# s-a-malik/fumi

Measured on AMD Instinct MI355X. Metric: episodes/sec (5-way 5-shot FuMI), higher is better.
Workload: dtype f32; 1 GPU; FuMI 5-way 5-shot, 32 query/class, ResNet-152-style 2048-d embeddings, im_hid [256,64], GloVe-300 token text (L=128, V=20000, mean pool), text_hid 256, 1 inner step, second-order meta-gradient + Adam step; BASELINE.json configs[1]; episodes_per_gpu=32, global_meta_batch=32, parallelism=episode-sharded x1, 1 all-reduce of the flat gradient

## Files before the change

fumi_amd/csrc/episode.hip:

```cpp
#include "common.h"
#include <algorithm>
#include <stdlib.h>

namespace {

unsigned long long* g_epi_trace = nullptr;
int g_spin_limit = 1 << 22;
constexpr int QR = 32;
constexpr int MAXL = FUMI_MAX_HIDDEN;

struct EpiBuf {
    float *A0, *G;
    float *D, *cs;
    float *bcur[MAXL], *bh;
    float *Wslot[MAXL], *Whslot;
    float *ta[MAXL], *tdz[MAXL], *tp, *te;
    float *lg;
    float *aq[MAXL], *zq[MAXL], *lbar, *qcs;
    float *pW[MAXL], *pb[MAXL], *pWh, *pbh, *pb0, *pD, *ploss, *pcorr;
    float *Wb[MAXL], *bb[MAXL], *Whb, *bhb, *b0b, *Db;
    float *abar[MAXL], *X0, *X1, *eb, *lb;
    float *A0bar;
    float *A0bar_q; int ldsr, ldq;
    float *apart; int *acnt;
// ... 950 lines not shown
    float* Whb = w.Whb + (long)b * N * H;
    float* bhb = w.bhb + (long)b * N;
    float* b0b = w.b0b + (long)b * h0;
    float* Db = w.Db + (long)b * S * h0;
    float* A0bs = w.A0bar + (long)b * w.ldsr * h0;
    auto sum_tiles = [&](float* dst, const float* src, long sz) {
        wg_sum_slabs(dst, src + (long)b * ntile * sz, ntile, sz, sz);
    };
    for (int i = 1; i < L; ++i) {
        const long sz = (long)d.h[i] * d.h[i - 1];
        sum_tiles(Wb(i), w.pW[i], sz);
        sum_tiles(bb(i), w.pb[i], d.h[i]);
    }
    sum_tiles(Whb, w.pWh, (long)N * H);
    sum_tiles(bhb, w.pbh, N);
    sum_tiles(b0b, w.pb0, h0);
    sum_tiles(Db, w.pD, (long)S * h0);
    for (int i = tid; i < S * h0; i += nt) A0bs[i] = 0.f;
    __syncthreads();

    if (d.second_order) {
        const float* Gss = w.G + (long)b * (S + d.Qn) * S;
        float* cs = w.cs + (long)b * h0;
        float* eb = w.eb + (long)b * S * N;
        float* lb = w.lb + (long)b * S * N;
        float* const Xa = w.X0 + (long)b * S * w.maxh;
        float* const Xb = w.X1 + (long)b * S * w.maxh;
        auto X = [&](int i) { return i ? Xb : Xa; };
        for (int t = d.T - 1; t >= 0; --t) {
            auto a = [&](int i) { return (const float*)(w.ta[i] + ((long)b * w.ntape + t) * S * d.h[i]); };
            auto dz = [&](int i) { return (const float*)(w.tdz[i] + ((long)b * w.ntape + t) * S * d.h[i]); };
            auto ab = [&](int i) { return w.abar[i] + (long)b * S * d.h[i]; };
            auto Wc = [&](int i) { return (const float*)(w.Wslot[i] + ((long)b * w.nslot + t) * ((long)d.h[i] * d.h[i - 1])); };
            const float* Whc = w.Whslot + ((long)b * w.nslot + t) * N * H;
            const float* p = w.tp + ((long)b * w.ntape + t) * S * N;
            const float* e = w.te + ((long)b * w.ntape + t) * S * N;

            for (int i = 0; i < L; ++i) {
                float* abi = ab(i);
                for (int j = tid; j < S * d.h[i]; j += nt) abi[j] = 0.f;
            }
            int cur = 0;
            {
                wg_ew((long)S * h0, Xa, a(0), Db, nullptr, [&](long, float m_, float v, float) { return m_ > 0.f ? v * d.mscale : 0.f; });
            }
            __syncthreads();
            for (int i = 1; i < L; ++i) {
                const int hi = d.h[i], hp = d.h[i - 1];
                const float* dab = X(cur); float* nxt = X(cur ^ 1);
                const float* bbi = bb(i); const float* Wbi = Wb(i); const float* ai = a(i);
                wg_mm2(sm, sm_cap, S, hi, hp, dab, hp, 1, Wc(i), 1, hp, [&](int m, int n) { return bbi[n]; },
                       [&](int m, int n, float acc, float pre) { nxt[(long)m * hi + n] = acc - alpha * pre; });
                wg_mm2(sm, sm_cap, S, hi, hp, a(i - 1), hp, 1, Wbi, 1, hp,
                       [&](int m, int n) { return f32pair{nxt[(long)m * hi + n], ai[(long)m * hi + n]}; },
                       [&](int m, int n, float acc, f32pair pre) {
                           nxt[(long)m * hi + n] = pre.y > 0.f ? (pre.x - alpha * acc) * d.mscale : 0.f;
                       });
                float* abp = ab(i - 1);
                wg_mm2(sm, sm_cap, S, hp, hi, dz(i), hi, 1, Wbi, hp, 1, [&](int m, int n) { return abp[(long)m * hp + n]; },
                       [&](int m, int n, float acc, float pre) { abp[(long)m * hp + n] = pre - alpha * acc; });
                __syncthreads();
                float* Wbw = Wb(i);
                wg_mm2(sm, sm_cap, hi, hp, S, dz(i), 1, hi, dab, hp, 1, [&](int m, int n) { return Wbw[(long)m * hp + n]; },
                       [&](int m, int n, float acc, float pre) { Wbw[(long)m * hp + n] = pre + acc; });
                __syncthreads();
                cur ^= 1;
            }
            {
                const float* dab = X(cur);
                wg_mm2(sm, sm_cap, S, N, H, dab, H, 1, Whc, 1, H, [&](int m, int n) { return bhb[n]; },
                       [&](int m, int n, float acc, float pre) { eb[m * N + n] = acc - alpha * pre; });
                wg_mm2(sm, sm_cap, S, N, H, a(L - 1), H, 1, Whb, 1, H, [&](int m, int n) { return eb[m * N + n]; },
                       [&](int m, int n, float acc, float pre) { eb[m * N + n] = pre - alpha * acc; });
                float* abl = ab(L - 1);
                wg_mm2(sm, sm_cap, S, H, N, e, N, 1, Whb, H, 1, [&](int m, int n) { return abl[(long)m * H + n]; },
                       [&](int m, int n, float acc, float pre) { abl[(long)m * H + n] = pre - alpha * acc; });
                __syncthreads();
                wg_mm2(sm, sm_cap, N, H, S, e, 1, N, dab, H, 1, [&](int m, int n) { return Whb[m * H + n]; },
                       [&](int m, int n, float acc, float pre) { Whb[m * H + n] = pre + acc; });
                for (int s = tid; s < S; s += nt) {
                    float dot = 0.f;
                    for (int n = 0; n < N; ++n) dot += p[s * N + n] * eb[s * N + n];
                    for (int n = 0; n < N; ++n) lb[s * N + n] = p[s * N + n] * (eb[s * N + n] - dot) / (float)S;
                }
                __syncthreads();
                wg_mm2(sm, sm_cap, S, H, N, lb, N, 1, Whc, H, 1, [&](int m, int n) { return abl[(long)m * H + n]; },
                       [&](int m, int n, float acc, float pre) { abl[(long)m * H + n] = pre + acc; });
                wg_mm2(sm, sm_cap, N, H, S, lb, 1, N, a(L - 1), H, 1, [&](int m, int n) { return Whb[m * H + n]; },
                       [&](int m, int n, float acc, float pre) { Whb[m * H + n] = pre + acc; });
                wg_colsum(sm, sm_cap, S, N, lb, N, [&](int n, float s) { bhb[n] += s; });
                __syncthreads();
            }
            for (int i = L - 1; i >= 1; --i) {
                const int hi = d.h[i], hp = d.h[i - 1];
                float* zb = ab(i);
                {
                    wg_ew((long)S * hi, zb, a(i), zb, nullptr, [&](long, float m_, float v, float) { return m_ > 0.f ? v * d.mscale : 0.f; });
                }
                __syncthreads();
                float* abp = ab(i - 1); float* Wbw = Wb(i); float* bbw = bb(i);
                wg_mm2(sm, sm_cap, S, hp, hi, zb, hi, 1, Wc(i), hp, 1, [&](int m, int n) { return abp[(long)m * hp + n]; },
                       [&](int m, int n, float acc, float pre) { abp[(long)m * hp + n] = pre + acc; });
                wg_mm2(sm, sm_cap, hi, hp, S, zb, 1, hi, a(i - 1), hp, 1, [&](int m, int n) { return Wbw[(long)m * hp + n]; },
                       [&](int m, int n, float acc, float pre) { Wbw[(long)m * hp + n] = pre + acc; });
                wg_colsum(sm, sm_cap, S, hi, zb, hi, [&](int n, float s) { bbw[n] += s; });
                __syncthreads();
            }
            float* z0b = ab(0);
            wg_ew((long)S * h0, z0b, a(0), z0b, nullptr, [&](long, float m_, float v, float) { return m_ > 0.f ? v * d.mscale : 0.f; });
            __syncthreads();
            wg_ew((long)S * h0, A0bs, A0bs, z0b, nullptr, [&](long, float x, float y, float) { return x + y; });
            __syncthreads();
            wg_colsum(sm, sm_cap, S, h0, z0b, h0, [&](int n, float s) { cs[n] = s; b0b[n] += s; });
            __syncthreads();
            wg_mm2(sm, sm_cap, S, h0, S, Gss, S, 1, z0b, h0, 1,
                   [&](int m, int n) { return f32pair{Db[(long)m * h0 + n], cs[n]}; },
                   [&](int m, int n, float acc, f32pair pre) { Db[(long)m * h0 + n] = pre.x - alpha * (acc + pre.y); });
            __syncthreads();
        }
    }
    float* hb = head_bar + (long)b * N * (H + 1);
    for (int j = tid; j < N * H; j += nt) hb[(j / H) * (H + 1) + (j % H)] = Whb[j];
    for (int j = tid; j < N; j += nt) hb[j * (H + 1) + H] = bhb[j];
}

constexpr int RLDS_CAP = 40000;
struct RLay {
    int Wb[MAXL], bb[MAXL], a[MAXL], dz[MAXL], W[MAXL], ab[MAXL];
    int Db, A0bs, b0b, Whb, bhb, Wh, p, e, eb, G, dab0, X0, X1, cs, ldX, total;
};
__host__ __device__ constexpr void reverse_layout(RLay& y, int L, const int* h, int S, int N, int P) {
    int off = 0;
    const int RS = q_r4(S), h0c = h[0] / P, H = h[L - 1];
    auto take = [&](int rows, int ld) { const int o = off; off += rows * ld; return o; };
    for (int i = 0; i < MAXL; ++i) y.Wb[i] = y.bb[i] = y.a[i] = y.dz[i] = y.W[i] = y.ab[i] = 0;
    int maxh1 = 4;
    for (int i = 1; i < L; ++i) maxh1 = h[i] > maxh1 ? h[i] : maxh1;
    y.ldX = wg_ld(maxh1);
    for (int i = 1; i < L; ++i) {
        const int kc = i == 1 ? h0c : h[i - 1];
        y.Wb[i] = take(q_r16(h[i]), wg_ld(kc)); y.W[i] = take(q_r16(h[i]), wg_ld(kc)); y.bb[i] = take(1, q_r4(h[i]));
        y.a[i] = take(RS, wg_ld(h[i])); y.dz[i] = take(RS, wg_ld(h[i])); y.ab[i] = take(RS, wg_ld(h[i]));
    }
    y.a[0] = take(RS, wg_ld(h0c)); y.ab[0] = take(RS, wg_ld(h0c)); y.dab0 = take(RS, wg_ld(h0c));
    y.Db = take(RS, wg_ld(h0c)); y.A0bs = take(RS, wg_ld(h0c));
    y.X0 = take(RS, y.ldX); y.X1 = take(RS, y.ldX);
    y.Whb = take(q_r16(N), wg_ld(H)); y.Wh = take(q_r16(N), wg_ld(H));
    y.p = take(RS, wg_ld(N)); y.e = take(RS, wg_ld(N)); y.eb = take(RS, wg_ld(N)); y.G = take(RS, wg_ld(S));
    y.b0b = take(1, q_r4(h0c)); y.cs = take(1, q_r4(h0c)); y.bhb = take(1, q_r4(N));
    y.total = off + 64;
}
constexpr RLay ref_rlay() { RLay y{}; const int h[MAXL] = {REF_H0, REF_H1}; reverse_layout(y, 2, h, REF_SP, REF_NP, REF_P); return y; }
static_assert(ref_qlay().total <= QLDS_CAP && ref_rlay().total <= RLDS_CAP, "the reference layouts fit the CU's LDS");

template <bool FIX = false, bool DROP = true>
__global__ __launch_bounds__(512) void reverse_lds_kernel(StageTab stg_init, StageTab stg_step, EpiDims d_arg, EpiBuf w, RLay y_arg,
                                                          int P_arg, float* loss_b, float* acc_b, float* head_bar) {
    EpiDims d_fix = d_arg; fix_dims<FIX, DROP>(d_fix);
    const EpiDims& d = FIX ? d_fix : d_arg;
    auto dh = [&](int i) { return FIX ? (i == 0 ? REF_H0 : REF_H1) : d_arg.h[i]; };
    RLay y_fix = y_arg;
    if constexpr (FIX) { constexpr RLay k = ref_rlay(); y_fix = k; }
    const RLay& y = FIX ? y_fix : y_arg;
    const int P = FIX ? REF_P : P_arg;
    extern __shared__ __attribute__((aligned(16))) float sm[];
    __shared__ StageTab s_stg[2];
    const int tid = threadIdx.x, nt = blockDim.x;
    const int xcd = blockIdx.x & 7, jq = blockIdx.x >> 3;
    const int b = xcd + 8 * (jq / P), c = jq % P;
    if (b >= d.B) return;
    int ri = 0;
#define RSTAMP() if (w.trace && tid == 0 && blockIdx.x == 0) w.trace[128 + ri++] = __builtin_amdgcn_s_memrealtime();
    RSTAMP()
    const int S = d.S, N = d.N, L = d.L, H = d.H, h0 = dh(0), h0c = h0 / P, c0 = c * h0c, h1 = dh(1);
    const float alpha = d.alpha, ms = d.mscale;
    const int ntile = w.ntile;
    if (tid == 0 && c == 0) {
        float ls = 0.f, cr = 0.f;
        for (int t = 0; t < ntile; ++t) { ls += w.ploss[(long)b * ntile + t]; cr += w.pcorr[(long)b * ntile + t]; }
        loss_b[b] = ls / (float)d.Qn;
        acc_b[b] = cr / (float)d.Qn;
    }
    if (!d.need_grad) return;

    const int ldc = wg_ld(h0c), ldN = wg_ld(N), ldS = wg_ld(S), ldH = wg_ld(H), ldX = y.ldX;
    auto ldh = [&](int i) { return wg_ld(dh(i)); };
    const f32x4 z4 = {0.f, 0.f, 0.f, 0.f};
    auto relu_bwd4 = [&](const f32x4& act, const f32x4& g) {
        f32x4 o;
#pragma unroll
        for (int e = 0; e < 4; ++e) o[e] = act[e] > 0.f ? g[e] * ms : 0.f;
        return o;
    };
    auto ew = [&](int cols, auto&& f) {
        const int c4n = (cols + 3) >> 2;
        for (int i = tid; i < S * c4n; i += nt) { const int m = i / c4n; f(m, (i - m * c4n) << 2); }
    };
    auto store_img = [&](float* dst, long drs, const float* img, int ld, int rows, int cols) {
        const int c4n = (cols + 3) >> 2;
        for (int i = tid; i < rows * c4n; i += nt) {
            const int r = i / c4n, cc = (i - r * c4n) << 2;
            wg_st4(dst + (long)r * drs + cc, *(const f32x4*)(img + r * ld + cc), min(4, cols - cc));
        }
    };

    wg_stage_tab_to_lds(s_stg, 2, (int)(2 * sizeof(StageTab) + sizeof(EpiDims) + sizeof(EpiBuf) + sizeof(RLay) + 64));
    for (int i = tid * 4, tot = y.total; i < tot; i += nt * 4) *(f32x4*)(sm + i) = z4;
    __syncthreads(); RSTAMP()
    wg_stage_rows<3, 8>(&s_stg[0], b, 0, c, 0, sm);
    wg_lds_barrier(); RSTAMP()

    float* Wb1 = sm + y.Wb[1]; float* Db = sm + y.Db; float* A0bs = sm + y.A0bs; float* b0b = sm + y.b0b;
    float* Whb = sm + y.Whb; float* bhb = sm + y.bhb; float* cs = sm + y.cs;
    float* a0 = sm + y.a[0]; float* ab0 = sm + y.ab[0]; float* dab0 = sm + y.dab0; float* W1 = sm + y.W[1];
    float* Wh = sm + y.Wh; float* pp = sm + y.p; float* ee = sm + y.e; float* eb = sm + y.eb; float* G = sm + y.G;
    float* Xa = sm + y.X0; float* Xb = sm + y.X1;

    if (d.second_order) {
        for (int t = d.T - 1; t >= 0; --t) {
            const int round = d.T - 1 - t;
            wg_stage_rows<8, 1>(&s_stg[1], b, t, c, 0, sm);
            wg_lds_barrier(); RSTAMP()
            for (int i = 1; i < L; ++i) { float* abi = sm + y.ab[i]; const int ldi = ldh(i); ew(dh(i), [&](int m, int n) { *(f32x4*)(abi + m * ldi + n) = z4; }); }
            ew(h0c, [&](int m, int n) {
                *(f32x4*)(ab0 + m * ldc + n) = z4;
                *(f32x4*)(dab0 + m * ldc + n) = relu_bwd4(*(const f32x4*)(a0 + m * ldc + n), *(const f32x4*)(Db + m * ldc + n));
            });
            wg_lds_barrier(); RSTAMP()
            const float* dz1 = sm + y.dz[1]; const int ld1 = ldh(1);
            wg_lmm<true, true>(S, h1, h0c, dab0, ldc, W1, ldc, [&](int m, int n, const f32x4& acc, int) { *(f32x4*)(Xa + m * ldX + n) = acc; });
            wg_lmm<true, true>(S, h1, h0c, a0, ldc, Wb1, ldc, [&](int m, int n, const f32x4& acc, int) {
                float* px = Xa + m * ldX + n; *(f32x4*)px = *(const f32x4*)px - alpha * acc;
            });
            wg_lmm_wide<true>(S, h0c, h1, dz1, ld1, Wb1, ldc, [&](int m, int n, const f32x4& acc, int, auto) {
                float* pa = ab0 + m * ldc + n; *(f32x4*)pa = *(const f32x4*)pa - alpha * acc;
            });
            wg_lds_barrier(); RSTAMP()
            float* xb = w.xpart + (((long)b * 2 + (round & 1)) * 8) * (long)S * h1;
            if (P > 1) {
                float* mine = xb + (long)c * S * h1;
                for (int i = tid; i < S * h1; i += nt) {
                    const int m = i / h1, n = i - m * h1;
                    __hip_atomic_store(mine + i, Xa[m * ldX + n], __ATOMIC_RELAXED, __HIP_MEMORY_SCOPE_AGENT);
                }
            }
            wg_lmm_wide<false>(h1, h0c, S, dz1, ld1, dab0, ldc, [&](int m, int n, const f32x4& acc, int, auto) {
                float* pw = Wb1 + m * ldc + n; *(f32x4*)pw = *(const f32x4*)pw + acc;
            });
            if (P > 1) {
                wg_drain_stores();
                __syncthreads();
                if (tid == 0) {
                    __hip_atomic_fetch_add(w.xcnt + b, 1, __ATOMIC_RELAXED, __HIP_MEMORY_SCOPE_AGENT);
                    const int target = P * (round + 1);
                    int spin = 0;
                    while (__hip_atomic_load(w.xcnt + b, __ATOMIC_RELAXED, __HIP_MEMORY_SCOPE_AGENT) < target) {
                        if (++spin > w.spin_limit) { atomicOr(w.status, FUMI_ST_SYNC_TIMEOUT); break; }
                        __builtin_amdgcn_s_sleep(2);
                    }
                }
                __syncthreads();
            } else {
                wg_lds_barrier();
            }
            RSTAMP()
            {
                const float* a1 = sm + y.a[1]; const float* bb1 = sm + y.bb[1];
                const int w4 = q_r4(h1);
                for (int i = tid; i < S * w4; i += nt) {
                    const int m = i / w4, n = i - m * w4;
                    float v = 0.f;
                    if (n < h1) {
                        if (P > 1) { for (int cc = 0; cc < P; ++cc) v += __hip_atomic_load(xb + (long)cc * S * h1 + m * h1 + n, __ATOMIC_RELAXED, __HIP_MEMORY_SCOPE_AGENT); }
                        else v = Xa[m * ldX + n];
                        v = a1[m * ld1 + n] > 0.f ? (v - alpha * bb1[n]) * ms : 0.f;
                    }
                    Xb[m * ldX + n] = v;
                }
            }
            wg_lds_barrier(); RSTAMP()
            int cur = 1;
            auto X = [&](int i) { return i ? Xb : Xa; };
            for (int i = 2; i < L; ++i) {
                const int hi = dh(i), hp = dh(i - 1), ldi = ldh(i), ldp = ldh(i - 1);
                const float* dab = X(cur); float* nxt = X(cur ^ 1);
                const float* bbi = sm + y.bb[i]; float* Wbi = sm + y.Wb[i]; const float* ai = sm + y.a[i];
                const float* dzi = sm + y.dz[i]; float* abp = sm + y.ab[i - 1];
                wg_lmm<true, true>(S, hi, hp, dab, ldX, sm + y.W[i], ldp, [&](int m, int n, const f32x4& acc, int) {
                    *(f32x4*)(nxt + m * ldX + n) = acc - alpha * *(const f32x4*)(bbi + n);
                });
                wg_lmm<true, true>(S, hi, hp, sm + y.a[i - 1], ldp, Wbi, ldp, [&](int m, int n, const f32x4& acc, int) {
                    float* px = nxt + m * ldX + n;
                    *(f32x4*)px = relu_bwd4(*(const f32x4*)(ai + m * ldi + n), *(const f32x4*)px - alpha * acc);
                });
                wg_lmm_wide<true>(S, hp, hi, dzi, ldi, Wbi, ldp, [&](int m, int n, const f32x4& acc, int, auto) {
                    float* pa = abp + m * ldp + n; *(f32x4*)pa = *(const f32x4*)pa - alpha * acc;
                });
                wg_lds_barrier();
                wg_lmm_wide<false>(hi, hp, S, dzi, ldi, dab, ldX, [&](int m, int n, const f32x4& acc, int, auto) {
                    float* pw = Wbi + m * ldp + n; *(f32x4*)pw = *(const f32x4*)pw + acc;
                });
                wg_lds_barrier();
                cur ^= 1;
            }
            {
                const float* dab = X(cur); const float* aL = sm + y.a[L - 1]; float* abl = sm + y.ab[L - 1];
                wg_lmm<true, true>(S, N, H, dab, ldX, Wh, ldH, [&](int m, int n, const f32x4& acc, int) {
                    *(f32x4*)(eb + m * ldN + n) = acc - alpha * *(const f32x4*)(bhb + n);
                });
                wg_lmm<true, true>(S, N, H, aL, ldH, Whb, ldH, [&](int m, int n, const f32x4& acc, int) {
                    float* pe = eb + m * ldN + n; *(f32x4*)pe = *(const f32x4*)pe - alpha * acc;
                });
                wg_lmm_wide<true>(S, H, N, ee, ldN, Whb, ldH, [&](int m, int n, const f32x4& acc, int, auto) {
                    float* pa = abl + m * ldH + n; *(f32x4*)pa = *(const f32x4*)pa - alpha * acc;
                });
                wg_lds_barrier(); RSTAMP()
                wg_lmm_wide<false>(N, H, S, ee, ldN, dab, ldX, [&](int m, int n, const f32x4& acc, int, auto) {
                    float* pw = Whb + m * ldH + n; *(f32x4*)pw = *(const f32x4*)pw + acc;
                });
                for (int s_ = tid; s_ < S; s_ += nt) {
                    float* re = eb + s_ * ldN; const float* rp = pp + s_ * ldN;
                    float dot = 0.f;
                    for (int n = 0; n < N; ++n) dot += rp[n] * re[n];
                    for (int n = 0; n < N; ++n) re[n] = rp[n] * (re[n] - dot) / (float)S;
                    for (int n = N; n < q_r4(N); ++n) re[n] = 0.f;
                }
                wg_lds_barrier(); RSTAMP()
                const float* lb = eb;
                wg_lmm_wide<true>(S, H, N, lb, ldN, Wh, ldH, [&](int m, int n, const f32x4& acc, int, auto) {
                    float* pa = abl + m * ldH + n; *(f32x4*)pa = *(const f32x4*)pa + acc;
                });
                wg_lmm_wide<false>(N, H, S, lb, ldN, aL, ldH, [&](int m, int n, const f32x4& acc, int, auto) {
                    float* pw = Whb + m * ldH + n; *(f32x4*)pw = *(const f32x4*)pw + acc;
                });
                wg_lcolsum(S, N, lb, ldN, [&](int n, float s_) { bhb[n] += s_; });
                wg_lds_barrier(); RSTAMP()
            }
            for (int i = L - 1; i >= 1; --i) {
                const int hi = dh(i), ldi = ldh(i);
                float* zb = sm + y.ab[i]; const float* ai = sm + y.a[i];
                ew(hi, [&](int m, int n) { float* pz = zb + m * ldi + n; *(f32x4*)pz = relu_bwd4(*(const f32x4*)(ai + m * ldi + n), *(const f32x4*)pz); });
                wg_lds_barrier();
                float* bbw = sm + y.bb[i];
                if (i >= 2) {
                    const int hp = dh(i - 1), ldp = ldh(i - 1);
                    float* abp = sm + y.ab[i - 1]; float* Wbi = sm + y.Wb[i];
                    wg_lmm_wide<true>(S, hp, hi, zb, ldi, sm + y.W[i], ldp, [&](int m, int n, const f32x4& acc, int, auto) {
                        float* pa = abp + m * ldp + n; *(f32x4*)pa = *(const f32x4*)pa + acc;
                    });
                    wg_lmm_wide<false>(hi, hp, S, zb, ldi, sm + y.a[i - 1], ldp, [&](int m, int n, const f32x4& acc, int, auto) {
                        float* pw = Wbi + m * ldp + n; *(f32x4*)pw = *(const f32x4*)pw + acc;
                    });
                } else {
                    wg_lmm_wide<true>(S, h0c, hi, zb, ldi, W1, ldc, [&](int m, int n, const f32x4& acc, int, auto) {
                        float* pa = ab0 + m * ldc + n; *(f32x4*)pa = *(const f32x4*)pa + acc;
                    });
                    wg_lmm_wide<false>(hi, h0c, S, zb, ldi, a0, ldc, [&](int m, int n, const f32x4& acc, int, auto) {
                        float* pw = Wb1 + m * ldc + n; *(f32x4*)pw = *(const f32x4*)pw + acc;
                    });
                }
                wg_lcolsum(S, hi, zb, ldi, [&](int n, float s_) { bbw[n] += s_; });
                wg_lds_barrier(); RSTAMP()
            }
            ew(h0c, [&](int m, int n) {
                float* pz = ab0 + m * ldc + n;
                const f32x4 z = relu_bwd4(*(const f32x4*)(a0 + m * ldc + n), *(const f32x4*)pz);
                *(f32x4*)pz = z;
                float* pA = A0bs + m * ldc + n; *(f32x4*)pA = *(const f32x4*)pA + z;
            });
            wg_lds_barrier();
            wg_lcolsum(S, h0c, ab0, ldc, [&](int n, float s_) { cs[n] = s_; b0b[n] += s_; });
            wg_lds_barrier();
            wg_lmm_wide<true>(S, h0c, S, G, ldS, ab0, ldc, [&](int m, int n, const f32x4& acc, int, auto) {
                float* pd = Db + m * ldc + n; *(f32x4*)pd = *(const f32x4*)pd - alpha * (acc + *(const f32x4*)(cs + n));
            });
            wg_lds_barrier(); RSTAMP()
        }
    }
    store_img(w.Wb[1] + (long)b * h1 * h0 + c0, h0, Wb1, ldc, h1, h0c);
    store_img(w.A0bar + (long)b * w.ldsr * h0 + c0, h0, A0bs, ldc, S, h0c);
    for (int n = tid; n < h0c; n += nt) w.b0b[(long)b * h0 + c0 + n] = b0b[n];
    if (c == 0) {
        for (int i = 1; i < L; ++i) {
            const float* bbi = sm + y.bb[i];
            for (int n = tid; n < dh(i); n += nt) w.bb[i][(long)b * dh(i) + n] = bbi[n];
            if (i >= 2) store_img(w.Wb[i] + (long)b * dh(i) * dh(i - 1), dh(i - 1), sm + y.Wb[i], ldh(i - 1), dh(i), dh(i - 1));
        }
        float* hb = head_bar + (long)b * N * (H + 1);
        for (int j = tid; j < N * H; j += nt) { const int n = j / H, k = j - n * H; hb[n * (H + 1) + k] = Whb[n * ldH + k]; }
        for (int j = tid; j < N; j += nt) hb[j * (H + 1) + H] = bhb[j];
    }
    RSTAMP()
#undef RSTAMP
}

__global__ void class_text_select_kernel(int N, int S, int Dt, const float* text_s, const int64_t* y_s, float* out,
                                         int* status) {
    const int b = blockIdx.y, n = blockIdx.x, lane = threadIdx.x;
    const int64_t* ys = y_s + (long)b * S;
    int first = S;
    for (int s0 = 0; s0 < S && first == S; s0 += 64) {
        const int s = s0 + lane;
        const bool hit = s < S && ys[s] == n;
        const unsigned long long m = __ballot(hit);
        if (m) first = s0 + __ffsll((long long)m) - 1;
    }
    float* o = out + ((long)b * N + n) * Dt;
    if (first == S) {
        if (lane == 0) atomicOr(status, FUMI_ST_CLASS_MISSING);
        for (int j = lane; j < Dt; j += 64) o[j] = __builtin_nanf("");
        return;
    }
    const float* src = text_s + ((long)b * S + first) * Dt;
    for (int j = lane; j < Dt; j += 64) o[j] = src[j];
}

__global__ void broadcast_head_kernel(int N, int H, const float* Wf, const float* bf, float* head) {
    float* hb = head + (long)blockIdx.x * N * (H + 1);
    for (int j = threadIdx.x; j < N * (H + 1); j += blockDim.x) {
        const int n = j / (H + 1), c = j % (H + 1);
        hb[j] = c < H ? Wf[n * H + c] : bf[n];
    }
}

__global__ void tanh_bwd_kernel(long n, const float* h, const float* hbar, float* out) {
    for (long i = blockIdx.x * (long)blockDim.x + threadIdx.x; i < n; i += (long)gridDim.x * blockDim.x)
        out[i] = hbar[i] * (1.f - h[i] * h[i]);
}

__global__ void relu_mask_mul_kernel(long n, const float* u, float* g, float scale) {
    for (long i = blockIdx.x * (long)blockDim.x + threadIdx.x; i < n; i += (long)gridDim.x * blockDim.x)
        g[i] = u[i] > 0.f ? g[i] * scale : 0.f;
}

__global__ void split_head_grad_kernel(int B, int N, int H, const float* head_bar, float scale, float* gW, float* gb) {
    const int j = blockIdx.x * blockDim.x + threadIdx.x;
    if (j >= N * (H + 1)) return;
    float s = 0.f;
    for (int b = 0; b < B; ++b) s += head_bar[(long)b * N * (H + 1) + j];
    const int n = j / (H + 1), c = j % (H + 1);
    if (c < H) gW[n * H + c] = scale * s; else gb[n] = scale * s;
}

template <auto K> struct KernTag { static constexpr auto fn = K; };

inline int blocks_for(long n) { long b = (n + 255) / 256; return (int)(b > 2048 ? 2048 : (b < 1 ? 1 : b)); }

struct Carver {
    fumi_ws* ws; size_t bytes;
    float* take(size_t n) {
        bytes += ws_align(n * sizeof(float));
        return ws ? ws_f(ws, n) : nullptr;
    }
};

void carve(Carver& c, const EpisodeProblem& p, EpiBuf& w) {
    const size_t B = p.B, S = p.S, Qn = p.Qn, N = p.N, L = p.L, h0 = p.h[0], H = p.h[L - 1];
    const bool taped = p.need_grad && p.second_order && p.T > 0;
    w.nslot = taped ? p.T + 1 : 1;
    w.ntape = taped ? p.T : 1;
    w.ntile = (p.Qn + QR - 1) / QR;
    int maxh = 0;
    for (int i = 0; i < p.L; ++i) maxh = p.h[i] > maxh ? p.h[i] : maxh;
    w.maxh = maxh;
    {
        auto r16 = [](int x) { return (x + 15) & ~15; };
        auto need = [&](int M, int N_, int K) { return (long)(r16(M) + 4 + r16(N_) + 4) * (r16(K) + 4); };
        const int S_ = p.S, N_ = p.N, H_ = p.h[p.L - 1], h0_ = p.h[0], R_ = QR;
        long a = need(S_, h0_, S_), q = need(R_, h0_, S_), r = need(S_, h0_, S_);
        a = std::max({a, need(S_, N_, H_), need(S_, H_, N_), need(N_, H_, S_)});
        q = std::max({q, need(R_, N_, H_), need(N_, H_, R_), need(R_, H_, N_), need(S_, h0_, R_)});
        r = std::max({r, need(S_, N_, H_), need(S_, H_, N_), need(N_, H_, S_)});
        for (int i = 1; i < p.L; ++i) {
            const int hi = p.h[i], hp = p.h[i - 1];
            a = std::max({a, need(S_, hi, hp), need(S_, hp, hi), need(hi, hp, S_)});
            q = std::max({q, need(R_, hi, hp), need(R_, hp, hi), need(hi, hp, R_)});
            r = std::max({r, need(S_, hi, hp), need(S_, hp, hi), need(hi, hp, S_)});
        }
        const long cap = 38000;
        w.lds_adapt = (int)std::min(a, cap); w.lds_query = (int)std::min(q, cap); w.lds_reverse = (int)std::min(r, cap);
    }
    const size_t nt = w.ntile;
    w.A0 = c.take(B * (S + Qn) * h0); w.G = c.take(B * (S + Qn) * S);
    w.D = c.take(B * S * h0); w.cs = c.take(B * h0);
    w.bh = c.take(B * N); w.Whslot = c.take(B * w.nslot * N * H);
    w.tp = c.take(B * w.ntape * S * N); w.te = c.take(B * w.ntape * S * N);
    w.lg = c.take(B * S * N);
    w.lbar = c.take(B * Qn * N); w.qcs = c.take(B * nt * h0);
    w.ploss = c.take(B * nt); w.pcorr = c.take(B * nt);
    w.apart = c.take(B * 2 * 8 * S * (L > 1 ? (size_t)p.h[1] : 1)); w.acnt = nullptr;
    for (size_t i = 0; i < L; ++i) {
        const size_t hi = p.h[i], hp = i ? p.h[i - 1] : 0;
        w.ta[i] = c.take(B * w.ntape * S * hi); w.tdz[i] = c.take(B * w.ntape * S * hi);
        w.aq[i] = c.take(B * Qn * hi); w.zq[i] = c.take(B * Qn * hi);
        if (i >= 1) { w.bcur[i] = c.take(B * hi); w.Wslot[i] = c.take(B * w.nslot * hi * hp); }
        else { w.bcur[i] = nullptr; w.Wslot[i] = nullptr; }
    }
    if (p.need_grad) {
        w.pWh = c.take(B * nt * N * H); w.pbh = c.take(B * nt * N); w.pb0 = c.take(B * nt * h0); w.pD = c.take(B * nt * S * h0);
        w.Whb = c.take(B * N * H); w.bhb = c.take(B * N); w.b0b = c.take(B * h0); w.Db = c.take(B * S * h0);
        w.X0 = c.take(B * S * maxh); w.X1 = c.take(B * S * maxh); w.eb = c.take(B * S * N); w.lb = c.take(B * S * N);
        w.A0bar = c.take(B * (S + Qn) * h0);
        w.xpart = c.take(B * 2 * 8 * S * (L > 1 ? (size_t)p.h[1] : 1)); w.xcnt = (int*)c.take(B);
        for (size_t i = 0; i < L; ++i) {
            const size_t hi = p.h[i], hp = i ? p.h[i - 1] : 0;
            w.abar[i] = c.take(B * S * hi);
            if (i >= 1) {
                w.pW[i] = c.take(B * nt * hi * hp); w.pb[i] = c.take(B * nt * hi);
                w.Wb[i] = c.take(B * hi * hp); w.bb[i] = c.take(B * hi);
            } else { w.pW[i] = w.pb[i] = w.Wb[i] = w.bb[i] = nullptr; }
        }
    }
}


}

void set_xpanel_trace(void* p);
void set_rn12_trace(void* p);
extern "C" int fumi_hip_set_trace_buffer(int which, void* p) {
    if (which == 0) g_epi_trace = (unsigned long long*)p;
    else if (which == 1) set_xpanel_trace(p);
    else if (which == 2) set_rn12_trace(p);
    else return FUMI_EINVAL;
    return FUMI_OK;
}
static int g_epi_fixed_last = 0;
extern "C" int fumi_hip_epi_fixed_last() { return g_epi_fixed_last; }
// ... 51 lines not shown

    if (p.inputs_ready) HIP_TRY(hipEventRecord(p.inputs_ready, st));
    {
        ProfScope ps(ws, st, FUMI_PH_XPANEL_FWD);
        int rider_done = 0;
        if ((rc = launch_xpanel_fwd(st, p.B, p.S, p.Qn, p.D, h0, p.x_s, p.x_q, p.W[0], w.A0, w.G, p.rows.table ? &p.rows : nullptr,
                                    p.fwd_rider, &rider_done, nullptr, nullptr, xpanel_planes(ws, p.B, p.S, p.D, h0), p.glove))) return rc;
        if (p.fwd_rider && !rider_done && p.fwd_rider_fallback && (rc = p.fwd_rider_fallback(p.hook_ctx))) return rc;
    }
    if (p.after_xpanel_fwd && (rc = p.after_xpanel_fwd(p.hook_ctx))) return rc;
    if (p.head_ready) HIP_TRY(hipStreamWaitEvent(st, p.head_ready, 0));
    EpiParams prm;
    for (int i = 0; i < MAXL; ++i) { prm.W[i] = i < p.L ? p.W[i] : nullptr; prm.b[i] = i < p.L ? p.b[i] : nullptr; }
    static const int fuse_env = getenv("FUMI_EPI_FUSE") ? atoi(getenv("FUMI_EPI_FUSE")) : 1;
    QLay qlf; StageTab tbq, tbs;
    bool fuse_q = fuse_env && !getenv("FUMI_EPI_GLOBAL") && p.T == 1 && p.L == 2 && p.S <= QR && (h0 & 3) == 0 && p.head != nullptr;
    static const int fixed_env = getenv("FUMI_EPI_FIXED") ? atoi(getenv("FUMI_EPI_FIXED")) : 1;
    const bool fixed = fixed_env && !getenv("FUMI_EPI_GLOBAL") && p.T == 1 && p.L == 2 && p.h[0] == REF_H0 && p.h[1] == REF_H1 &&
                       p.S <= REF_SP && p.N <= REF_NP && p.need_grad && p.second_order;
    bool fixed_q = fixed && fuse_q && p.S <= REF_SQ;
    g_epi_fixed_last = 0;
    const bool drop = d.drop_thr != 0;
    if (fuse_q) {
        if (fixed_q) qlf = ref_qlay();
        else query_layout(qlf, p.L, p.h, p.S, p.N, true);
        fuse_q = qlf.total <= QLDS_CAP;
    }
    if (fuse_q) {
        const long R = p.S + p.Qn, S = p.S, N = p.N, H = d.H;
        const int h1 = p.h[1];
        tbs.init(); tbq.init();
        tbs.add(w.A0, R * h0, 0, 0, h0, p.S, p.S, h0, qlf.a[0], wg_ld(h0));
        tbs.add(p.W[1], 0, 0, 0, h0, h1, h1, h0, qlf.W[1], wg_ld(h0));
        tbs.add(p.b[1], 0, 0, 0, h1, 1, 1, h1, qlf.bi[1], h1);
        tbs.add(p.head, N * (H + 1), 0, 0, H + 1, p.N, p.N, (int)H, qlf.Wh, wg_ld((int)H));
        tbs.add(p.head + H, N * (H + 1), 0, 0, H + 1, p.N, p.N, 1, qlf.bh, 1);
        tbs.add(p.b[0], 0, 0, 0, h0, 1, 1, h0, qlf.b0, h0);
        tbs.add(w.G + S * S, R * S, (long)QR * S, 0, S, -1, QR, p.S, qlf.Gq, wg_ld(p.S));
        fuse_q = !tbs.bad && tbs.nunits <= 64 * 8 && h0 <= 256;
        auto a16 = [](const void* q) { return (((uintptr_t)q) & 15) == 0; };
        fixed_q = fixed_q && a16(p.W[1]) && a16(p.b[1]) && a16(p.b[0]);
    }
    if (!fuse_q) {
        ProfScope ps(ws, st, FUMI_PH_ADAPT);
        static const bool force_global_a = getenv("FUMI_EPI_GLOBAL") != nullptr;
        static const int ap_env = getenv("FUMI_ADAPT_P") ? atoi(getenv("FUMI_ADAPT_P")) : 1;
        int AP = 1;
        if (ap_env > 1 && p.L >= 2 && w.acnt && p.B <= FUMI_ACNT) {
            AP = ap_env > 8 ? 8 : ap_env;
            while (AP > 1 && (h0 % (64 * AP) != 0)) AP >>= 1;
        }
        int hs[MAXL];
        for (int i = 0; i < MAXL; ++i) hs[i] = i < p.L ? p.h[i] : 0;
        hs[0] = h0 / AP;
        ALay al; adapt_layout(al, p.L, hs, p.S, p.N);
        const int H = d.H;
        bool lds_form = al.total <= ALDS_CAP && 4 + 2 * (p.L - 1) <= WG_MAXJOB && !force_global_a &&
                        ((p.S + 15) / 16) * ((hs[0] + 63) / 64) <= 8;
        StageTab tb; tb.init();
        if (lds_form) {
            const long R = p.S + p.Qn, S = p.S, N = p.N;
            tb.add(w.G, R * S, 0, 0, S, p.S, p.S, p.S, al.G, wg_ld(p.S));
            for (int i = 1; i < p.L; ++i) {
                const int kc = i == 1 ? hs[0] : p.h[i - 1];
                tb.add(p.W[i], 0, 0, i == 1 ? hs[0] : 0, p.h[i - 1], p.h[i], p.h[i], kc, al.W[i], wg_ld(kc));
                tb.add(p.b[i], 0, 0, 0, p.h[i], 1, 1, p.h[i], al.bi[i], p.h[i]);
            }
            tb.add(p.head, N * (H + 1), 0, 0, H + 1, p.N, p.N, H, al.Wh, wg_ld(H));
            tb.add(p.head + H, N * (H + 1), 0, 0, H + 1, p.N, p.N, 1, al.bh, 1);
            lds_form = !tb.bad && tb.nunits <= 64 * 8;
        }
        if (lds_form) {
            FUMI_SET_DYN_LDS(adapt_lds_kernel, al.total * 4);
            const unsigned grid = AP > 1 ? 8u * ((p.B + 7) / 8) * AP : (unsigned)p.B;
            hipLaunchKernelGGL(adapt_lds_kernel, dim3(grid), dim3(512), al.total * 4, st, tb, d, w, al, prm, p.y_s, ws->status, AP);
        } else {
            FUMI_SET_DYN_LDS(adapt_kernel, w.lds_adapt * 4);
            hipLaunchKernelGGL(adapt_kernel, dim3(p.B), dim3(512), w.lds_adapt * 4, st, d, w, prm, p.y_s, p.head, ws->status);
        }
        LAUNCH_CHECK();
    }
    if (fuse_q) {
        ProfScope ps(ws, st, FUMI_PH_QUERY);
        auto launch = [&](auto tag) -> int {
            constexpr auto kern = decltype(tag)::fn;
            FUMI_SET_DYN_LDS(kern, qlf.total * 4);
            hipLaunchKernelGGL(kern, dim3(w.ntile, p.B), dim3(512), qlf.total * 4, st, tbq, tbs, d, w, qlf, p.y_q,
                               p.logits_q, p.preds_q, p.preds_f, ws->status, p.y_s);
            LAUNCH_CHECK();
            return FUMI_OK;
        };
        if (fixed_q) g_epi_fixed_last |= 1;
        if (fixed_q) rc = drop ? launch(KernTag<query_lds_kernel<true, true, true>>{}) : launch(KernTag<query_lds_kernel<true, true, false>>{});
        else rc = launch(KernTag<query_lds_kernel<true>>{});
        if (rc) return rc;
    } else {
        ProfScope ps(ws, st, FUMI_PH_QUERY);
        QLay ql; query_layout(ql, p.L, p.h, p.S, p.N);
        static const bool force_global = getenv("FUMI_EPI_GLOBAL") != nullptr;
        bool lds_form = ql.total <= QLDS_CAP && 7 + 2 * (p.L - 1) <= WG_MAXJOB && !force_global;
        StageTab tb; tb.init();
        if (lds_form) {
            const long R = p.S + p.Qn, S = p.S, N = p.N, H = d.H;
            const long slot = d.taped ? p.T : 0;
            tb.add(w.A0 + S * h0, R * h0, (long)QR * h0, 0, h0, -1, QR, h0, ql.a[0], wg_ld(h0));
            tb.add(w.D, S * h0, 0, 0, h0, p.S, p.S, h0, ql.D, wg_ld(h0));
            for (int i = 1; i < p.L; ++i) {
                const long sz = (long)p.h[i] * p.h[i - 1];
                tb.add(w.Wslot[i] + slot * sz, w.nslot * sz, 0, 0, p.h[i - 1], p.h[i], p.h[i], p.h[i - 1], ql.W[i], wg_ld(p.h[i - 1]));
            }
            tb.add(w.G + S * S, R * S, (long)QR * S, 0, S, -1, QR, p.S, ql.Gq, wg_ld(p.S));
            tb.add(w.Whslot + slot * N * H, w.nslot * N * H, 0, 0, H, p.N, p.N, (int)H, ql.Wh, wg_ld((int)H));
            tb.add(p.b[0], 0, 0, 0, h0, 1, 1, h0, ql.b0, h0);
            tb.add(w.cs, h0, 0, 0, h0, 1, 1, h0, ql.cs, h0);
            for (int i = 1; i < p.L; ++i) tb.add(w.bcur[i], p.h[i], 0, 0, p.h[i], 1, 1, p.h[i], ql.bi[i], p.h[i]);
            tb.add(w.bh, N, 0, 0, N, 1, 1, p.N, ql.bh, p.N);
            lds_form = !tb.bad && tb.nunits <= 64 * 8;
        }
        if (lds_form) {
            StageTab none; none.init();
            FUMI_SET_DYN_LDS(query_lds_kernel<false>, ql.total * 4);
            hipLaunchKernelGGL(query_lds_kernel<false>, dim3(w.ntile, p.B), dim3(512), ql.total * 4, st, tb, none, d, w, ql, p.y_q,
                               p.logits_q, p.preds_q, p.preds_f, ws->status, p.y_s);
        } else {
            FUMI_SET_DYN_LDS(query_kernel, w.lds_query * 4);
            hipLaunchKernelGGL(query_kernel, dim3(w.ntile, p.B), dim3(512), w.lds_query * 4, st, d, w, p.b[0], p.y_q, p.logits_q,
                               p.preds_q, p.preds_f, ws->status);
        }
        LAUNCH_CHECK();
    }
    if (two_part) {
        xpanel_bwd_two_part_split(p.B, p.S, p.Qn, p.D, h0, &nsq, &kcq, &nss, &kcs);
        const long slab = (long)h0 * p.D;
        bwd_slabs = ws_f(ws, (size_t)(nsq + nss) * slab);
        HIP_TRY(hipEventRecord(ws->evx[0], st));
        HIP_TRY(hipStreamWaitEvent(ws->side, ws->evx[0], 0));
        if ((rc = launch_xpanel_bwd(ws->side, p.B, 0, p.Qn, p.D, h0, nullptr, p.x_q, w.A0bar_q, bwd_slabs, kcq, nsq,
                                    p.rows.table ? &p.rows : nullptr, nullptr, nullptr))) return rc;
        HIP_TRY(hipEventRecord(ws->evx[1], ws->side));
    }
    {
        ProfScope ps(ws, st, FUMI_PH_REVERSE);
        static const bool force_global_r = getenv("FUMI_EPI_GLOBAL") != nullptr;
        bool lds_form = p.L >= 2 && p.L <= 4 && w.ntile <= 8 && !force_global_r;
        int P = 0; RLay rl; StageTab ti, tsx;
        if (lds_form) {
            for (int cand = 1; cand <= 8 && !P; cand *= 2) {
                if (h0 % (4 * cand)) break;
                reverse_layout(rl, p.L, p.h, p.S, p.N, cand);
                if (rl.total <= RLDS_CAP) P = cand;
            }
            lds_form = P > 0;
        }
        const bool fixed_r = fixed && lds_form && P == REF_P;
        if (fixed_r) rl = ref_rlay();
        if (lds_form) {
            const long S = p.S, N = p.N, H = d.H, R = p.S + p.Qn, nt = w.ntile, h0c = h0 / P, h1 = p.h[1];
            ti.init(); tsx.init();
            ti.add(w.pW[1], nt * h1 * h0, 0, h0c, h0, (int)h1, (int)h1, (int)h0c, rl.Wb[1], wg_ld((int)h0c), (int)nt, h1 * h0);
            ti.add(w.pD, nt * S * h0, 0, h0c, h0, p.S, p.S, (int)h0c, rl.Db, wg_ld((int)h0c), (int)nt, S * h0);
            ti.add(w.pb0, nt * h0, 0, h0c, h0, 1, 1, (int)h0c, rl.b0b, (int)h0c, (int)nt, h0);
            ti.add(w.pWh, nt * N * H, 0, 0, H, p.N, p.N, (int)H, rl.Whb, wg_ld((int)H), (int)nt, N * H);
            ti.add(w.pbh, nt * N, 0, 0, N, 1, 1, p.N, rl.bhb, p.N, (int)nt, N);
            for (int i = 1; i < p.L; ++i) {
                const long hi = p.h[i], hp = p.h[i - 1];
                ti.add(w.pb[i], nt * hi, 0, 0, hi, 1, 1, (int)hi, rl.bb[i], (int)hi, (int)nt, hi);
                if (i >= 2) ti.add(w.pW[i], nt * hi * hp, 0, 0, hp, (int)hi, (int)hi, (int)hp, rl.Wb[i], wg_ld((int)hp), (int)nt, hi * hp);
            }
            ti.add(w.G, R * S, 0, 0, S, p.S, p.S, p.S, rl.G, wg_ld(p.S));
            tsx.add(w.ta[0], w.ntape * S * h0, S * h0, h0c, h0, p.S, p.S, (int)h0c, rl.a[0], wg_ld((int)h0c));
            tsx.add(w.Wslot[1], w.nslot * h1 * h0, h1 * h0, h0c, h0, (int)h1, (int)h1, (int)h0c, rl.W[1], wg_ld((int)h0c));
            for (int i = 1; i < p.L; ++i) {
                const long hi = p.h[i], hp = p.h[i - 1];
                tsx.add(w.ta[i], w.ntape * S * hi, S * hi, 0, hi, p.S, p.S, (int)hi, rl.a[i], wg_ld((int)hi));
                tsx.add(w.tdz[i], w.ntape * S * hi, S * hi, 0, hi, p.S, p.S, (int)hi, rl.dz[i], wg_ld((int)hi));
                if (i >= 2) tsx.add(w.Wslot[i], w.nslot * hi * hp, hi * hp, 0, hp, (int)hi, (int)hi, (int)hp, rl.W[i], wg_ld((int)hp));
            }
            tsx.add(w.Whslot, w.nslot * N * H, N * H, 0, H, p.N, p.N, (int)H, rl.Wh, wg_ld((int)H));
            tsx.add(w.tp, w.ntape * S * N, S * N, 0, N, p.S, p.S, p.N, rl.p, wg_ld(p.N));
            tsx.add(w.te, w.ntape * S * N, S * N, 0, N, p.S, p.S, p.N, rl.e, wg_ld(p.N));
            lds_form = !ti.bad && !tsx.bad && ti.nunits <= 64 * 8 && tsx.nunits <= 64 * 8;
        }
        if (lds_form) {
            auto launch = [&](auto tag) -> int {
                constexpr auto kern = decltype(tag)::fn;
                FUMI_SET_DYN_LDS(kern, rl.total * 4);
                hipLaunchKernelGGL(kern, dim3(8 * ((p.B + 7) / 8) * P), dim3(512), rl.total * 4, st, ti, tsx, d, w, rl, P,
                                   p.loss_b, p.acc_b, p.head_bar);
                LAUNCH_CHECK();
                return FUMI_OK;
            };
            if (fixed_r) g_epi_fixed_last |= 2;
            if (fixed_r) rc = drop ? launch(KernTag<reverse_lds_kernel<true, true>>{}) : launch(KernTag<reverse_lds_kernel<true, false>>{});
            else rc = launch(KernTag<reverse_lds_kernel<>>{});
            if (rc) return rc;
        } else {
            FUMI_SET_DYN_LDS(reverse_kernel, w.lds_reverse * 4);
            hipLaunchKernelGGL(reverse_kernel, dim3(p.B), dim3(512), w.lds_reverse * 4, st, d, w, p.loss_b, p.acc_b, p.head_bar);
        }
        LAUNCH_CHECK();
    }
    if (p.after_reverse) HIP_TRY(hipEventRecord(p.after_reverse, st));
    {
        ProfScope pr(ws, st, FUMI_PH_REDUCE);
        ReduceSegs own; own.n = 0; own.scale = p.grad_scale;
        const bool defer = p.defer_reduce && p.need_grad && p.defer_reduce->n + 4 + 2 * p.L <= 24;
        ReduceSegs& sg = defer ? *p.defer_reduce : own;
        if (defer) sg.scale = p.grad_scale;
        if (p.stats) { sg.add(p.loss_b, p.B, 1, 1, p.stats); sg.add(p.acc_b, p.B, 1, 1, p.stats + 1); }
        if (p.need_grad) {
            for (int i = 1; i < p.L; ++i) {
                const long sz = (long)p.h[i] * p.h[i - 1];
                sg.add(w.Wb[i], p.B, sz, sz, p.gW[i]);
                sg.add(w.bb[i], p.B, p.h[i], p.h[i], p.gb[i]);
            }
            sg.add(w.b0b, p.B, h0, h0, p.gb[0]);
        }
        if (!defer && (rc = launch_reduce_multi(st, own))) return rc;
    }
    if (!p.need_grad) return FUMI_OK;
    {
        ProfScope pg(ws, st, FUMI_PH_XPANEL_BWD);
        int kc;
        int ns = xpanel_bwd_nsplit(p.B, p.S, p.Qn, p.D, h0, &kc);
        const long slab = (long)h0 * p.D;
        float* slabs = two_part ? bwd_slabs : ws_f(ws, (size_t)ns * slab);
        int rider_done = 0;
        if (two_part) {
            if ((rc = launch_xpanel_bwd(st, p.B, p.S, 0, p.D, h0, p.x_s, nullptr, w.A0bar, bwd_slabs + (size_t)nsq * slab, kcs, nss,
                                        p.rows.table ? &p.rows : nullptr, p.bwd_rider, &rider_done))) return rc;
            HIP_TRY(hipStreamWaitEvent(st, ws->evx[1], 0));
            ns = nsq + nss;
        } else
        if ((rc = launch_xpanel_bwd(st, p.B, p.S, p.Qn, p.D, h0, p.x_s, p.x_q, w.A0bar, slabs, kc, ns, p.rows.table ? &p.rows : nullptr,
                                    p.bwd_rider, &rider_done))) return rc;
        if (p.bwd_rider && !rider_done && p.bwd_rider_fallback && (rc = p.bwd_rider_fallback(p.hook_ctx2))) return rc;
        if (p.defer_reduce && p.defer_reduce->n < 24 && p.defer_reduce->scale == p.grad_scale) p.defer_reduce->add(slabs, ns, slab, slab, p.gW[0]);
        else if ((rc = launch_reduce_slabs(st, slabs, ns, slab, slab, p.grad_scale, p.gW[0]))) return rc;
    }
    return FUMI_OK;
}

int launch_class_text_select(hipStream_t st, int B, int N, int S, int Dt, const float* text_s, const int64_t* y_s,
                             float* out, int* status) {
    hipLaunchKernelGGL(class_text_select_kernel, dim3(N, B), dim3(64), 0, st, N, S, Dt, text_s, y_s, out, status);
    LAUNCH_CHECK();
    return FUMI_OK;
}
int launch_broadcast_head(hipStream_t st, int B, int N, int H, const float* Wf, const float* bf, float* head) {
    hipLaunchKernelGGL(broadcast_head_kernel, dim3(B), dim3(256), 0, st, N, H, Wf, bf, head);
    LAUNCH_CHECK();
    return FUMI_OK;
}
int launch_tanh_bwd(hipStream_t st, long n, const float* h, const float* hbar, float* out) {
    hipLaunchKernelGGL(tanh_bwd_kernel, dim3(blocks_for(n)), dim3(256), 0, st, n, h, hbar, out);
    LAUNCH_CHECK();
    return FUMI_OK;
}
int launch_relu_mask_mul(hipStream_t st, long n, const float* u, float* g, float scale) {
    hipLaunchKernelGGL(relu_mask_mul_kernel, dim3(blocks_for(n)), dim3(256), 0, st, n, u, g, scale);
    LAUNCH_CHECK();
    return FUMI_OK;
}
int launch_split_head_grad(hipStream_t st, int B, int N, int H, const float* head_bar, float scale, float* gW, float* gb) {
    hipLaunchKernelGGL(split_head_grad_kernel, dim3((N * (H + 1) + 255) / 256), dim3(256), 0, st, B, N, H, head_bar, scale, gW, gb);
    LAUNCH_CHECK();
    return FUMI_OK;
}
```

Before: 160,500 episodes/s.

## Stage reverse-sweep inputs via fixed-address register loads in the specialised kernel

In the fixed-shape reverse kernel, the table-driven staging is replaced by direct per-lane float4 loads. Each lane issues its loads, sums the tile partials in registers, and writes into the reference LDS layout, so the loads can be in flight while LDS is being zeroed. The ReLU backward for dab0 is folded into this staging, and the per-step restage and the trailing Db update are dropped for the fixed path, on the assumption of a single inner step. Host dispatch now also checks 16-byte alignment and ntile<=8, and static_asserts pin the layout. The cost is code that only works for one specific layout and step count.

```diff
diff --git a/fumi_amd/csrc/episode.hip b/fumi_amd/csrc/episode.hip
--- a/fumi_amd/csrc/episode.hip
+++ b/fumi_amd/csrc/episode.hip
@@ -1126,6 +1126,16 @@
 }
 constexpr RLay ref_rlay() { RLay y{}; const int h[MAXL] = {REF_H0, REF_H1}; reverse_layout(y, 2, h, REF_SP, REF_NP, REF_P); return y; }
 static_assert(ref_qlay().total <= QLDS_CAP && ref_rlay().total <= RLDS_CAP, "the reference layouts fit the CU's LDS");
+constexpr bool ref_rlay_ok() {
+    constexpr RLay y = ref_rlay();
+    const int v4[] = {y.Wb[1], y.W[1], y.bb[1], y.a[1], y.dz[1], y.ab[1], y.a[0], y.ab[0], y.dab0, y.Db, y.A0bs, y.Whb, y.Wh, y.b0b};
+    for (int o : v4) if (o & 3) return false;
+    return wg_ld(REF_H0 / REF_P) == 68 && wg_ld(REF_H1) == 68 && wg_ld(REF_NP) == 36 && y.ldX == 68 && (y.total & 3) == 0 &&
+           y.Wb[1] == 0 && y.W[1] == 64 * 68 && y.a[0] - y.ab[1] == REF_SP * 68 && y.Whb - y.X1 == REF_SP * 68 &&
+           y.bhb + q_r4(REF_NP) + 64 == y.total;
+}
+static_assert(ref_rlay_ok(), "the fixed-address staging of the reverse sweep assumes this layout");
+static_assert(REF_SP * REF_NP <= 512 && REF_NP * 16 <= 128, "one lane per staged element of p / e and per float4 of the head");
 
 template <bool FIX = false, bool DROP = true>
 __global__ __launch_bounds__(512) void reverse_lds_kernel(StageTab stg_init, StageTab stg_step, EpiDims d_arg, EpiBuf w, RLay y_arg,
@@ -1178,11 +1188,76 @@
         }
     };
 
-    wg_stage_tab_to_lds(s_stg, 2, (int)(2 * sizeof(StageTab) + sizeof(EpiDims) + sizeof(EpiBuf) + sizeof(RLay) + 64));
-    for (int i = tid * 4, tot = y.total; i < tot; i += nt * 4) *(f32x4*)(sm + i) = z4;
-    __syncthreads(); RSTAMP()
-    wg_stage_rows<3, 8>(&s_stg[0], b, 0, c, 0, sm);
-    wg_lds_barrier(); RSTAMP()
+    wg_stage_tab_to_lds(s_stg, FIX ? 0 : 2, (int)(2 * sizeof(StageTab) + sizeof(EpiDims) + sizeof(EpiBuf) + sizeof(RLay) + 64));
+    if constexpr (FIX) {
+        static_assert(REF_H0 / REF_P == 64 && REF_H1 == 64 && REF_SP <= 32 && REF_NP <= 8, "one float4 per lane and 32-row pass");
+        constexpr int LD = wg_ld(64), LDN = wg_ld(REF_NP);
+        const int r = tid >> 4, c4 = (tid & 15) << 2;
+        const bool rS = r < S;
+        const long rc = rS ? r : 0;
+        const long ntl = ntile;
+        auto sum_tiles = [&](const float* p, long ss) {
+            f32x4 tk[8];
+#pragma unroll
+            for (int k = 0; k < 8; ++k) tk[k] = *(const f32x4*)(p + (k < ntile ? k : 0) * ss);
+            f32x4 t = tk[0];
+#pragma unroll
+            for (int k = 1; k < 8; ++k) if (k < ntile) t += tk[k];
+            return t;
+        };
+        const float* pW1 = w.pW[1] + ((long)b * ntl * REF_H1 + r) * REF_H0 + c0 + c4;
+        const f32x4 vWb0 = sum_tiles(pW1, (long)REF_H1 * REF_H0), vWb1 = sum_tiles(pW1 + 32 * REF_H0, (long)REF_H1 * REF_H0);
+        const f32x4 vDb = sum_tiles(w.pD + ((long)b * ntl * S + rc) * REF_H0 + c0 + c4, (long)S * REF_H0);
+        const int sj = tid < 128 ? 0 : tid < 144 ? 1 : tid < 160 ? 2 : 3;
+        const bool sok = sj == 0 ? r < N : sj < 3;
+        const float* sp = sj == 1 ? w.pb0 + (long)b * ntl * REF_H0 + c0 + c4
+                        : sj == 2 ? w.pb[1] + (long)b * ntl * REF_H1 + c4
+                                  : w.pWh + ((long)b * ntl * N + (sj == 0 && r < N ? r : 0)) * REF_H1 + c4;
+        const long sss = sj == 1 ? REF_H0 : sj == 2 ? REF_H1 : (long)N * REF_H1;
+        const f32x4 vsm = sum_tiles(sp, sss);
+        const int nb = tid - 160;
+        const bool bok = nb >= 0 && nb < N;
+        float vbh;
+        {
+            const float* p = w.pbh + (long)b * ntl * N + (bok ? nb : 0);
+            float tk[8];
+#pragma unroll
+            for (int k = 0; k < 8; ++k) tk[k] = p[(k < ntile ? k : 0) * (long)N];
+            vbh = tk[0];
+#pragma unroll
+            for (int k = 1; k < 8; ++k) if (k < ntile) vbh += tk[k];
+        }
+        const f32x4 va0 = *(const f32x4*)(w.ta[0] + ((long)b * S + rc) * REF_H0 + c0 + c4);
+        const float* pWs = w.Wslot[1] + ((long)b * 2 * REF_H1 + r) * REF_H0 + c0 + c4;
+        const f32x4 vW0 = *(const f32x4*)pWs, vW1 = *(const f32x4*)(pWs + 32 * REF_H0);
+        const f32x4 va1 = *(const f32x4*)(w.ta[1] + ((long)b * S + rc) * REF_H1 + c4);
+        const f32x4 vdz = *(const f32x4*)(w.tdz[1] + ((long)b * S + rc) * REF_H1 + c4);
+        const f32x4 vWh = *(const f32x4*)(w.Whslot + ((long)b * 2 * N + (r < N ? r : 0)) * REF_H1 + c4);
+        const bool pok = tid < S * N;
+        const long pi = (long)b * S * N + (pok ? tid : 0);
+        const float vp = w.tp[pi], ve = w.te[pi];
+        for (int i = tid * 4, tot = y.total; i < tot; i += nt * 4) *(f32x4*)(sm + i) = z4;
+        wg_lds_barrier(); RSTAMP()
+        *(f32x4*)(sm + y.Wb[1] + r * LD + c4) = vWb0; *(f32x4*)(sm + y.Wb[1] + (r + 32) * LD + c4) = vWb1;
+        *(f32x4*)(sm + y.W[1] + r * LD + c4) = vW0; *(f32x4*)(sm + y.W[1] + (r + 32) * LD + c4) = vW1;
+        if (rS) {
+            *(f32x4*)(sm + y.Db + r * LD + c4) = vDb;
+            *(f32x4*)(sm + y.a[0] + r * LD + c4) = va0;
+            *(f32x4*)(sm + y.dab0 + r * LD + c4) = relu_bwd4(va0, vDb);
+            *(f32x4*)(sm + y.a[1] + r * LD + c4) = va1;
+            *(f32x4*)(sm + y.dz[1] + r * LD + c4) = vdz;
+        }
+        if (sok) *(f32x4*)(sm + (sj == 0 ? y.Whb + r * LD : sj == 1 ? y.b0b : y.bb[1]) + c4) = vsm;
+        if (bok) sm[y.bhb + nb] = vbh;
+        if (r < N) *(f32x4*)(sm + y.Wh + r * LD + c4) = vWh;
+        if (pok) { const int m = tid / N, n = tid - m * N; sm[y.p + m * LDN + n] = vp; sm[y.e + m * LDN + n] = ve; }
+        wg_lds_barrier(); RSTAMP()
+    } else {
+        for (int i = tid * 4, tot = y.total; i < tot; i += nt * 4) *(f32x4*)(sm + i) = z4;
+        __syncthreads(); RSTAMP()
+        wg_stage_rows<3, 8>(&s_stg[0], b, 0, c, 0, sm);
+        wg_lds_barrier(); RSTAMP()
+    }
 
     float* Wb1 = sm + y.Wb[1]; float* Db = sm + y.Db; float* A0bs = sm + y.A0bs; float* b0b = sm + y.b0b;
     float* Whb = sm + y.Whb; float* bhb = sm + y.bhb; float* cs = sm + y.cs;
@@ -1193,6 +1268,7 @@
     if (d.second_order) {
         for (int t = d.T - 1; t >= 0; --t) {
             const int round = d.T - 1 - t;
+            if constexpr (!FIX) {
             wg_stage_rows<8, 1>(&s_stg[1], b, t, c, 0, sm);
             wg_lds_barrier(); RSTAMP()
             for (int i = 1; i < L; ++i) { float* abi = sm + y.ab[i]; const int ldi = ldh(i); ew(dh(i), [&](int m, int n) { *(f32x4*)(abi + m * ldi + n) = z4; }); }
@@ -1201,6 +1277,7 @@
                 *(f32x4*)(dab0 + m * ldc + n) = relu_bwd4(*(const f32x4*)(a0 + m * ldc + n), *(const f32x4*)(Db + m * ldc + n));
             });
             wg_lds_barrier(); RSTAMP()
+            }
             const float* dz1 = sm + y.dz[1]; const int ld1 = ldh(1);
             wg_lmm<true, true>(S, h1, h0c, dab0, ldc, W1, ldc, [&](int m, int n, const f32x4& acc, int) { *(f32x4*)(Xa + m * ldX + n) = acc; });
             wg_lmm<true, true>(S, h1, h0c, a0, ldc, Wb1, ldc, [&](int m, int n, const f32x4& acc, int) {
@@ -1343,11 +1420,15 @@
                 float* pA = A0bs + m * ldc + n; *(f32x4*)pA = *(const f32x4*)pA + z;
             });
             wg_lds_barrier();
+            if constexpr (FIX) {
+                wg_lcolsum(S, h0c, ab0, ldc, [&](int n, float s_) { b0b[n] += s_; });
+            } else {
             wg_lcolsum(S, h0c, ab0, ldc, [&](int n, float s_) { cs[n] = s_; b0b[n] += s_; });
             wg_lds_barrier();
             wg_lmm_wide<true>(S, h0c, S, G, ldS, ab0, ldc, [&](int m, int n, const f32x4& acc, int, auto) {
                 float* pd = Db + m * ldc + n; *(f32x4*)pd = *(const f32x4*)pd - alpha * (acc + *(const f32x4*)(cs + n));
             });
+            }
             wg_lds_barrier(); RSTAMP()
         }
     }
@@ -1705,7 +1786,9 @@
             }
             lds_form = P > 0;
         }
-        const bool fixed_r = fixed && lds_form && P == REF_P;
+        auto a16r = [](const void* q) { return (((uintptr_t)q) & 15) == 0; };
+        const bool fixed_r = fixed && lds_form && P == REF_P && w.ntile <= 8 && a16r(w.pW[1]) && a16r(w.pD) && a16r(w.pb0) && a16r(w.pWh) &&
+                             a16r(w.pb[1]) && a16r(w.ta[0]) && a16r(w.ta[1]) && a16r(w.tdz[1]) && a16r(w.Wslot[1]) && a16r(w.Whslot);
         if (fixed_r) rl = ref_rlay();
         if (lds_form) {
             const long S = p.S, N = p.N, H = d.H, R = p.S + p.Qn, nt = w.ntile, h0c = h0 / P, h1 = p.h[1];
```

New measurement: 165,100 episodes/s (median of 6 runs). 1.03x the previous value.
